# arangesh/TrackMPNN

Hardware: AMD Instinct MI355X
Metric: graph_edges_per_sec_fwd_bwd (higher is better)
Workload: dtype f32; 1 GPU; C2 KITTI Car/RRC-shaped rolling windows: 7 frames, D_t~clip(Poisson(6),1,20), F=8 (2d), H=64, K=0, diff; 1 fwd per frame + 1 bwd per window; 16384 windows/GPU batched block-diagonally (64 distinct seeds tiled); windows_per_gpu=16384, rows_final=6762496, parallelism=sequence-dp1

## Files before the change

### trackmpnn_amd/csrc/gru_fwd.hip

```cpp
#include "gru_common.h"

namespace tmpnn {

template <int CT, int XMODE>
__global__ __launch_bounds__(256, 2) void k_gru_fwd(GruFwdArgs a) {
    const int wave = threadIdx.x >> 6, lane = threadIdx.x & 63;
    const int c = lane & 31, half = lane >> 5;
    const int r0 = (blockIdx.x * 4 + wave) * 32;
    if (r0 >= a.R) return;
    const int H = a.H, H3 = 3 * a.H;
    const int col0 = blockIdx.y * (32 * CT);
    const int li = min(r0 + c, a.R - 1);
    const int row = a.rows[li];

    f32x16 acc_r[CT], acc_z[CT], acc_in[CT], acc_hn[CT];
#pragma unroll
    for (int t = 0; t < CT; ++t)
#pragma unroll
        for (int i = 0; i < 16; ++i) { acc_r[t][i] = 0.f; acc_z[t][i] = 0.f; acc_in[t][i] = 0.f; acc_hn[t][i] = 0.f; }

    for (int kt = 0; kt < a.IN / 32; ++kt) {
        const int f0 = kt * 32 + half * 16;
        float av[16];
        load_x16<XMODE>(a, li, row, f0, av);
// ... 463 lines not shown
    float* sBias = reinterpret_cast<float*>(next_item + 4);
    for (int i = threadIdx.x; i < 32; i += WPB * 64) {
        const int f = cw0 + i;
        sBias[i] = a.b_ih[f] + a.b_hh[f];
        sBias[32 + i] = a.b_ih[H + f] + a.b_hh[H + f];
        sBias[64 + i] = a.b_ih[2 * H + f];
        sBias[96 + i] = a.b_hh[2 * H + f];
        sBias[128 + i] = a.logit_part ? a.w_head[f] : 0.f;
    }
    if (threadIdx.x == 0) *next_item = 0;
    __syncthreads();
    const int wave = threadIdx.x >> 6, lane = threadIdx.x & 63;
    const int c = lane & 31, half = lane >> 5;
    if ((__builtin_amdgcn_readfirstlane(wave) >> 2) == 0) __builtin_amdgcn_s_setprio(2);
    const int tiles_total = (a.R + 31) / 32;
    const int per_group = (tiles_total + ngroups - 1) / ngroups;
    const int item_lo = group * per_group;
    const int item_hi = min(tiles_total, item_lo + per_group);

    int item = 0;
    if (lane == 0) item = atomicAdd(next_item, 1);
    item = __builtin_amdgcn_readfirstlane(item) + item_lo;
    if (item >= item_hi) return;
    int r0 = item * 32;
    int li = min(r0 + c, a.R - 1);
    int row = a.rows[li];
    float4 rawx[NQ4], rawh[NQ4];
    {
        const float4* xr = reinterpret_cast<const float4*>(a.msg + (size_t)(a.msg_compact ? li : row) * a.ld_msg + (H / 2) * half);
        const float4* hr = reinterpret_cast<const float4*>(a.h + (size_t)row * a.ld_h + (H / 2) * half);
#pragma unroll
        for (int i = 0; i < NQ4; ++i) rawx[i] = xr[i];
#pragma unroll
        for (int i = 0; i < NQ4; ++i) rawh[i] = hr[i];
    }
    float* stg = stg_base + wave * (32 * STG_LD);
    const uint16_t* wpi = sWi + c * KP + (H / 2) * half;
    const uint16_t* wph = sWh + c * KP + (H / 2) * half;

    for (;;) {
        int nitem = 0;
        if (lane == 0) nitem = atomicAdd(next_item, 1);
        nitem = __builtin_amdgcn_readfirstlane(nitem) + item_lo;
        const bool nvalid = nitem < item_hi;
        const int nr0 = nvalid ? nitem * 32 : r0;
        const int nli = min(nr0 + c, a.R - 1);
        const int nrow = a.rows[nli];
        f32x16 acc_r, acc_z, acc_hn, acc_in;
#pragma unroll
        for (int i = 0; i < 16; ++i) { acc_r[i] = 0.f; acc_z[i] = 0.f; acc_hn[i] = 0.f; acc_in[i] = 0.f; }
        Split8 b[NKB];
#pragma unroll
        for (int kb = 0; kb < NKB; ++kb) b[kb] = split8(rawx[2 * kb], rawx[2 * kb + 1]);
        if (nvalid) {
            const float4* xr = reinterpret_cast<const float4*>(a.msg + (size_t)(a.msg_compact ? nli : nrow) * a.ld_msg + (H / 2) * half);
#pragma unroll
            for (int i = 0; i < NQ4; ++i) rawx[i] = xr[i];
        }
#pragma unroll
        for (int kb = 0; kb < NKB; ++kb) {
#pragma unroll
            for (int g = 0; g < 3; ++g) {
                const uint16_t* wp = wpi + (g * 32) * KP + 8 * kb;
                const uint4 w1 = *reinterpret_cast<const uint4*>(wp);
                const uint4 w2 = *reinterpret_cast<const uint4*>(wp + NC * KP);
                const uint4 w3 = *reinterpret_cast<const uint4*>(wp + 2 * NC * KP);
                if (g == 0) acc_r = mfma_x6(w1, w2, w3, b[kb], acc_r);
                else if (g == 1) acc_z = mfma_x6(w1, w2, w3, b[kb], acc_z);
                else acc_in = mfma_x6(w1, w2, w3, b[kb], acc_in);
            }
        }
#pragma unroll
        for (int kb = 0; kb < NKB; ++kb) b[kb] = split8(rawh[2 * kb], rawh[2 * kb + 1]);
        if (nvalid) {
            const float4* hr = reinterpret_cast<const float4*>(a.h + (size_t)nrow * a.ld_h + (H / 2) * half);
#pragma unroll
            for (int i = 0; i < NQ4; ++i) rawh[i] = hr[i];
        }
#pragma unroll
        for (int kb = 0; kb < NKB; ++kb) {
#pragma unroll
            for (int g = 0; g < 3; ++g) {
                const uint16_t* wp = wph + (g * 32) * KP + 8 * kb;
                const uint4 w1 = *reinterpret_cast<const uint4*>(wp);
                const uint4 w2 = *reinterpret_cast<const uint4*>(wp + NC * KP);
                const uint4 w3 = *reinterpret_cast<const uint4*>(wp + 2 * NC * KP);
                if (g == 0) acc_r = mfma_x6(w1, w2, w3, b[kb], acc_r);
                else if (g == 1) acc_z = mfma_x6(w1, w2, w3, b[kb], acc_z);
                else acc_hn = mfma_x6(w1, w2, w3, b[kb], acc_hn);
            }
        }
        float4 hp4[4];
#pragma unroll
        for (int q = 0; q < 4; ++q)
            hp4[q] = *reinterpret_cast<const float4*>(a.h + (size_t)row * a.ld_h + cw0 + 8 * q + 4 * half);
        f32x16 outv;
#pragma unroll
        for (int q = 0; q < 4; ++q) {
            const float4 br = *reinterpret_cast<const float4*>(sBias + 8 * q + 4 * half);
            const float4 bz = *reinterpret_cast<const float4*>(sBias + 32 + 8 * q + 4 * half);
            const float4 bi = *reinterpret_cast<const float4*>(sBias + 64 + 8 * q + 4 * half);
            const float4 bh = *reinterpret_cast<const float4*>(sBias + 96 + 8 * q + 4 * half);
            const float brv[4] = {br.x, br.y, br.z, br.w}, bzv[4] = {bz.x, bz.y, bz.z, bz.w};
            const float biv[4] = {bi.x, bi.y, bi.z, bi.w}, bhv[4] = {bh.x, bh.y, bh.z, bh.w};
            const float hp[4] = {hp4[q].x, hp4[q].y, hp4[q].z, hp4[q].w};
#pragma unroll
            for (int i = 0; i < 4; ++i) {
                const int reg = 4 * q + i;
                const float ro = sigmoidf_(acc_r[reg] + brv[i]);
                const float zo = sigmoidf_(acc_z[reg] + bzv[i]);
                const float ho = acc_hn[reg] + bhv[i];
                const float no = tanhf_(acc_in[reg] + biv[i] + ro * ho);
                outv[reg] = (1.0f - zo) * no + zo * hp[i];
                acc_r[reg] = ro; acc_z[reg] = zo; acc_hn[reg] = ho; acc_in[reg] = no;
            }
        }
        if (a.logit_part) {
            float p = 0.f;
#pragma unroll
            for (int q = 0; q < 4; ++q) {
                const float4 w = *reinterpret_cast<const float4*>(sBias + 128 + 8 * q + 4 * half);
                p += outv[4 * q] * w.x + outv[4 * q + 1] * w.y + outv[4 * q + 2] * w.z + outv[4 * q + 3] * w.w;
            }
            p += __shfl_xor(p, 32);
            if (half == 0 && r0 + c < a.R) a.logit_part[(size_t)cwb * a.part_stride + row] = p;
        }
        stage_store32(stg, c, half, lane, outv, a.h_out, a.ld_out, cw0, row, r0, a.R);
        if (a.gates) {
            stage_store32<true>(stg, c, half, lane, acc_r, a.gates, H, cw0, row, r0, a.R);
            stage_store32<true>(stg, c, half, lane, acc_z, a.gates + a.gate_plane, H, cw0, row, r0, a.R);
            stage_store32<true>(stg, c, half, lane, acc_in, a.gates + 2 * a.gate_plane, H, cw0, row, r0, a.R);
            stage_store32<true>(stg, c, half, lane, acc_hn, a.gates + 3 * a.gate_plane, H, cw0, row, r0, a.R);
        }
        if (!nvalid) break;
        r0 = nr0; li = nli; row = nrow;
    }
}

#define FT_MARK(i) do { } while (0)
struct FwdTiles { const int32_t* t_row; const int32_t* t_loc; const int32_t* t_dptr; const int32_t* t_dets; int T; int zs_hn; };
static constexpr int TCAP = 24, TP_LD = 100;
static constexpr int TP_AREA = TCAP * TP_LD;

__device__ __forceinline__ uint32_t lds_addr_g(const void* p) {
    return (uint32_t)(uintptr_t)(const __attribute__((address_space(3))) char*)(const char*)p;
}
__device__ __forceinline__ void glds16_g(const void* gsrc, uint32_t lds_wave_base) {
    unsigned keep;
    lds_wave_base = __builtin_amdgcn_readfirstlane(lds_wave_base);
    asm volatile("s_mov_b32 %0, m0\n\ts_mov_b32 m0, %2\n\ts_nop 0\n\tglobal_load_lds_dwordx4 %1, off\n\ts_mov_b32 m0, %0"
                 : "=&s"(keep) : "v"(gsrc), "s"(lds_wave_base) : "memory");
}

struct TiledIdx { int row, loc, det, nd; };
__device__ __forceinline__ TiledIdx tiled_idx(const FwdTiles& tl, int R, int t, int c, int lane) {
    TiledIdx x;
    const int li = min(32 * t + c, R - 1);
    x.row = tl.t_row[li];
    x.loc = tl.t_loc[li];
    const int dp0 = tl.t_dptr[t];
    x.nd = tl.t_dptr[t + 1] - dp0;
    x.det = lane < x.nd ? tl.t_dets[dp0 + lane] : 0;
    return x;
}
template <int H>
__device__ __forceinline__ void tiled_stage_p(const GruFwdArgs& a, const TiledIdx& x, int cw0, int lane, uint32_t area) {
    const int nchunk = x.nd * 25;
#pragma unroll 1
    for (int i0 = 0; i0 < nchunk; i0 += 64) {
        const int idx = i0 + lane;
        const int j = idx / 25, rem = idx - 25 * j;
        const int j0 = i0 / 25;
        const int d0 = __builtin_amdgcn_readlane(x.det, j0), d1 = __builtin_amdgcn_readlane(x.det, j0 + 1);
        const int d2 = __builtin_amdgcn_readlane(x.det, j0 + 2), d3 = __builtin_amdgcn_readlane(x.det, min(j0 + 3, 63));
        const int dj = j - j0;
        const int det = dj == 0 ? d0 : dj == 1 ? d1 : dj == 2 ? d2 : d3;
        if (idx < nchunk && rem < 24)
            glds16_g(a.msg + (size_t)det * a.ld_msg + (rem >> 3) * H + cw0 + 4 * (rem & 7), area + 16u * i0);
    }
}

template <int H>
__device__ __forceinline__ void tiled_stage_p2(const GruFwdArgs& a, const TiledIdx& x, int cw0, int lane, uint32_t area) {
    const int sub = lane >= 25 ? 1 : 0, rem = lane - 25 * sub;
    const int goff = (rem >> 3) * H + cw0 + 4 * (rem & 7);
    const bool lane_on = rem < 24 && lane < 49;
#pragma unroll 1
    for (int k = 0; 2 * k < x.nd; ++k) {
        const int d0 = __builtin_amdgcn_readlane(x.det, 2 * k), d1 = __builtin_amdgcn_readlane(x.det, min(2 * k + 1, 63));
        const int det = sub ? d1 : d0;
        if (lane_on && 2 * k + sub < x.nd) glds16_g(a.msg + (size_t)det * a.ld_msg + goff, area + 800u * k);
    }
}

#define FT_STAGE_P tiled_stage_p2
template <int H, int WPB, bool ZS = false>
__global__ __launch_bounds__(WPB * 64, ZS ? 3 : 1) void k_gru_fwd_split_tiled(GruFwdArgs a, FwdTiles tl) {
    extern __shared__ float lds[];
    constexpr int H3 = 3 * H, KP = H + 8, NKB = H / 16, CW = H / 32, NQ4 = H / 8;
    uint16_t* sW = reinterpret_cast<uint16_t*>(lds);
    if constexpr (!ZS)
    for (int i = threadIdx.x; i < H * H3 / 4; i += WPB * 64) {
        const int k = i / (H3 / 4), j0 = (i % (H3 / 4)) * 4;
        const float4 w = *reinterpret_cast<const float4*>(a.whh_t + (size_t)k * H3 + j0);
        const float wv[4] = {w.x, w.y, w.z, w.w};
#pragma unroll
        for (int e = 0; e < 4; ++e) {
            uint16_t q1, q2, q3;
            split1(wv[e], q1, q2, q3);
            sW[(0 * H3 + j0 + e) * KP + k] = q1;
            sW[(1 * H3 + j0 + e) * KP + k] = q2;
            sW[(2 * H3 + j0 + e) * KP + k] = q3;
        }
    }
    float* area_base = reinterpret_cast<float*>(sW + (ZS ? 0 : 3 * H3 * KP));
    int* next_item = reinterpret_cast<int*>(area_base + WPB * TP_AREA);
    float* sBias = reinterpret_cast<float*>(next_item + 4);
    for (int i = threadIdx.x; i < H; i += WPB * 64) {
        sBias[i] = a.b_ih[i] + a.b_hh[i];
        sBias[H + i] = a.b_ih[H + i] + a.b_hh[H + i];
        sBias[2 * H + i] = a.b_ih[2 * H + i];
        sBias[3 * H + i] = a.b_hh[2 * H + i];
        sBias[4 * H + i] = a.logit_part ? a.w_head[i] : 0.f;
    }
    if (threadIdx.x == 0) *next_item = 0;
    __syncthreads();
    const int wave = threadIdx.x >> 6, lane = threadIdx.x & 63;
    const int c = lane & 31, half = lane >> 5;
    {
        const int grp = __builtin_amdgcn_readfirstlane(wave) >> 2;
        if (grp == 0) __builtin_amdgcn_s_setprio(3);
        else if (grp == 1) __builtin_amdgcn_s_setprio(2);
        else if (grp == 2) __builtin_amdgcn_s_setprio(1);
    }
    const int items_total = tl.T * CW;
    const int per_block = (items_total + gridDim.x - 1) / gridDim.x;
    const int item_lo = blockIdx.x * per_block;
    const int item_hi = min(items_total, item_lo + per_block);

    int item = 0;
    if (lane == 0) item = atomicAdd(next_item, 1);
    item = __builtin_amdgcn_readfirstlane(item) + item_lo;
    if (item >= item_hi) return;
    int cw0 = (item % CW) * 32;
    int t = item / CW;
    TiledIdx ix = tiled_idx(tl, a.R, t, c, lane);
    float* stg = area_base + wave * TP_AREA;
    const uint32_t area = lds_addr_g(stg);
    if (ix.nd <= TCAP) FT_STAGE_P<H>(a, ix, cw0, lane, area);
    float4 raw[NQ4];
    if constexpr (!ZS) {
        const float4* xr = reinterpret_cast<const float4*>(a.h + (size_t)ix.row * a.ld_h + (H / 2) * half);
#pragma unroll
        for (int i = 0; i < NQ4; ++i) raw[i] = xr[i];
    }

    for (;;) {
        int nitem = 0;
        if (lane == 0) nitem = atomicAdd(next_item, 1);
        nitem = __builtin_amdgcn_readfirstlane(nitem) + item_lo;
        const bool nvalid = nitem < item_hi;
        const int ncw0 = (nitem % CW) * 32;
        const int nt = nvalid ? nitem / CW : t;
        const int r0 = 32 * t;
        const int row = ix.row;
        const bool staged = ix.nd <= TCAP;
        Split8 b[NKB];
        if constexpr (!ZS) {
#pragma unroll
            for (int kb = 0; kb < NKB; ++kb) b[kb] = split8(raw[2 * kb], raw[2 * kb + 1]);
        }
        const TiledIdx nix = tiled_idx(tl, a.R, nt, c, lane);
        if constexpr (!ZS) {
            if (nvalid) {
                const float4* xr = reinterpret_cast<const float4*>(a.h + (size_t)nix.row * a.ld_h + (H / 2) * half);
#pragma unroll
                for (int i = 0; i < NQ4; ++i) raw[i] = xr[i];
            }
        }
        f32x16 acc_r, acc_z, acc_hn, acc_in;
#pragma unroll
        for (int i = 0; i < 16; ++i) { acc_r[i] = 0.f; acc_z[i] = 0.f; acc_hn[i] = 0.f; }
        if constexpr (!ZS) {
            const uint16_t* wp0 = sW + (cw0 + c) * KP + (H / 2) * half;
#pragma unroll
            for (int kb = 0; kb < NKB; ++kb) {
                const uint16_t* wp = wp0 + 8 * kb;
#pragma unroll
                for (int g = 0; g < 3; ++g) {
                    const uint4 w1 = *reinterpret_cast<const uint4*>(wp + (g * H) * KP);
                    const uint4 w2 = *reinterpret_cast<const uint4*>(wp + (H3 + g * H) * KP);
                    const uint4 w3 = *reinterpret_cast<const uint4*>(wp + (2 * H3 + g * H) * KP);
                    if (g == 0) acc_r = mfma_x6(w1, w2, w3, b[kb], acc_r);
                    else if (g == 1) acc_z = mfma_x6(w1, w2, w3, b[kb], acc_z);
                    else acc_hn = mfma_x6(w1, w2, w3, b[kb], acc_hn);
                }
            }
        }
        if (staged) {
            if (!ZS && nvalid) {
                if constexpr (NQ4 == 8) asm volatile("s_waitcnt vmcnt(8)" ::: "memory");
                else asm volatile("s_waitcnt vmcnt(4)" ::: "memory");
            } else {
                asm volatile("s_waitcnt vmcnt(0)" ::: "memory");
            }
        }
        float4 hp4[4];
        if constexpr (ZS) {
#pragma unroll
            for (int q = 0; q < 4; ++q) hp4[q] = make_float4(0.f, 0.f, 0.f, 0.f);
        } else {
#pragma unroll
            for (int q = 0; q < 4; ++q)
                hp4[q] = *reinterpret_cast<const float4*>(a.h + (size_t)row * a.ld_h + cw0 + 8 * q + 4 * half);
        }
        f32x16 outv;
        {
            float4 gs[4], gd[4], hs[4], hd[4];
            const int ls = ix.loc & 0xFFFF, ld_ = ix.loc >> 16;
            const int sdet = __shfl(ix.det, ls, 64), ddet = __shfl(ix.det, ld_, 64);
            const float* ps0 = a.msg + (size_t)sdet * a.ld_msg + cw0 + 4 * half;
            const float* pd0 = a.msg + (size_t)ddet * a.ld_msg + cw0 + 4 * half;
            if (staged) {
                const float* ls0 = stg + ls * TP_LD + 4 * half;
                const float* ld0 = stg + ld_ * TP_LD + 4 * half;
#pragma unroll
                for (int q = 0; q < 4; ++q) gs[q] = *reinterpret_cast<const float4*>(ls0 + 8 * q);
#pragma unroll
                for (int q = 0; q < 4; ++q) gd[q] = *reinterpret_cast<const float4*>(ld0 + 8 * q);
#pragma unroll
                for (int q = 0; q < 4; ++q) hs[q] = *reinterpret_cast<const float4*>(ls0 + 32 + 8 * q);
#pragma unroll
                for (int q = 0; q < 4; ++q) hd[q] = *reinterpret_cast<const float4*>(ld0 + 32 + 8 * q);
            } else {
#pragma unroll
                for (int q = 0; q < 4; ++q) gs[q] = *reinterpret_cast<const float4*>(ps0 + 8 * q);
#pragma unroll
                for (int q = 0; q < 4; ++q) gd[q] = *reinterpret_cast<const float4*>(pd0 + 8 * q);
#pragma unroll
                for (int q = 0; q < 4; ++q) hs[q] = *reinterpret_cast<const float4*>(ps0 + H + 8 * q);
#pragma unroll
                for (int q = 0; q < 4; ++q) hd[q] = *reinterpret_cast<const float4*>(pd0 + H + 8 * q);
            }
            __builtin_amdgcn_sched_barrier(0);
#pragma unroll
            for (int q = 0; q < 4; ++q) {
                const float4 b4 = *reinterpret_cast<const float4*>(sBias + cw0 + 8 * q + 4 * half);
                acc_r[4 * q + 0] = acc_r[4 * q + 0] + (gs[q].x - gd[q].x) + b4.x;
                acc_r[4 * q + 1] = acc_r[4 * q + 1] + (gs[q].y - gd[q].y) + b4.y;
                acc_r[4 * q + 2] = acc_r[4 * q + 2] + (gs[q].z - gd[q].z) + b4.z;
                acc_r[4 * q + 3] = acc_r[4 * q + 3] + (gs[q].w - gd[q].w) + b4.w;
            }
            __builtin_amdgcn_sched_barrier(0);
            if (staged) {
                const float* ls0 = stg + ls * TP_LD + 4 * half + 64;
                const float* ld0 = stg + ld_ * TP_LD + 4 * half + 64;
#pragma unroll
                for (int q = 0; q < 4; ++q) gs[q] = *reinterpret_cast<const float4*>(ls0 + 8 * q);
#pragma unroll
                for (int q = 0; q < 4; ++q) gd[q] = *reinterpret_cast<const float4*>(ld0 + 8 * q);
            } else {
#pragma unroll
                for (int q = 0; q < 4; ++q) gs[q] = *reinterpret_cast<const float4*>(ps0 + 2 * H + 8 * q);
#pragma unroll
                for (int q = 0; q < 4; ++q) gd[q] = *reinterpret_cast<const float4*>(pd0 + 2 * H + 8 * q);
            }
            __builtin_amdgcn_sched_barrier(0);
#pragma unroll
            for (int q = 0; q < 4; ++q) {
                const float4 b4 = *reinterpret_cast<const float4*>(sBias + H + cw0 + 8 * q + 4 * half);
                acc_z[4 * q + 0] = acc_z[4 * q + 0] + (hs[q].x - hd[q].x) + b4.x;
                acc_z[4 * q + 1] = acc_z[4 * q + 1] + (hs[q].y - hd[q].y) + b4.y;
                acc_z[4 * q + 2] = acc_z[4 * q + 2] + (hs[q].z - hd[q].z) + b4.z;
                acc_z[4 * q + 3] = acc_z[4 * q + 3] + (hs[q].w - hd[q].w) + b4.w;
            }
#pragma unroll
            for (int q = 0; q < 4; ++q) {
                const float4 b4 = *reinterpret_cast<const float4*>(sBias + 2 * H + cw0 + 8 * q + 4 * half);
                acc_in[4 * q + 0] = (gs[q].x - gd[q].x) + b4.x;
                acc_in[4 * q + 1] = (gs[q].y - gd[q].y) + b4.y;
                acc_in[4 * q + 2] = (gs[q].z - gd[q].z) + b4.z;
                acc_in[4 * q + 3] = (gs[q].w - gd[q].w) + b4.w;
            }
#pragma unroll
            for (int q = 0; q < 4; ++q) {
                const float4 b4h = *reinterpret_cast<const float4*>(sBias + 3 * H + cw0 + 8 * q + 4 * half);
                const float bh[4] = {b4h.x, b4h.y, b4h.z, b4h.w};
                const float hp[4] = {hp4[q].x, hp4[q].y, hp4[q].z, hp4[q].w};
#pragma unroll
                for (int i = 0; i < 4; ++i) {
                    const int reg = 4 * q + i;
                    const float ro = sigmoidf_(acc_r[reg]);
                    const float zo = sigmoidf_(acc_z[reg]);
                    const float ho = acc_hn[reg] + bh[i];
                    const float no = tanhf_(gru_n_preact(acc_in[reg], ro, ho));
                    outv[reg] = (1.0f - zo) * no + zo * hp[i];
                    acc_r[reg] = ro; acc_z[reg] = zo; acc_hn[reg] = ho; acc_in[reg] = no;
                }
            }
        }
        if (a.logit_part) {
            float p = 0.f;
#pragma unroll
            for (int q = 0; q < 4; ++q) {
                const float4 w = *reinterpret_cast<const float4*>(sBias + 4 * H + cw0 + 8 * q + 4 * half);
                p += outv[4 * q] * w.x + outv[4 * q + 1] * w.y + outv[4 * q + 2] * w.z + outv[4 * q + 3] * w.w;
            }
            p += __shfl_xor(p, 32);
            if (half == 0 && r0 + c < a.R) a.logit_part[(size_t)(cw0 / 32) * a.part_stride + row] = p;
        }
        asm volatile("s_waitcnt lgkmcnt(0)" ::: "memory");
        stage_store32(stg, c, half, lane, outv, a.h_out, a.ld_out, cw0, row, r0, a.R);
        if (a.gates) {
            stage_store32<true>(stg, c, half, lane, acc_r, a.gates, H, cw0, row, r0, a.R);
            stage_store32<true>(stg, c, half, lane, acc_z, a.gates + a.gate_plane, H, cw0, row, r0, a.R);
            stage_store32<true>(stg, c, half, lane, acc_in, a.gates + 2 * a.gate_plane, H, cw0, row, r0, a.R);
            if (!ZS || tl.zs_hn) stage_store32<true>(stg, c, half, lane, acc_hn, a.gates + 3 * a.gate_plane, H, cw0, row, r0, a.R);
        }
        if (!nvalid) break;
        cw0 = ncw0; t = nt; ix = nix;
        if (ix.nd <= TCAP) FT_STAGE_P<H>(a, ix, cw0, lane, area);
    }
}


static constexpr int T16_CAP = 12;
static constexpr int T16_AREA = T16_CAP * TP_LD;

__device__ __forceinline__ f32x4 mfma16_x6(const uint4& a1, const uint4& a2, const uint4& a3, const Split8& b, f32x4 c) {
    c = __builtin_amdgcn_mfma_f32_16x16x32_bf16(__builtin_bit_cast(bf16x8, a3), __builtin_bit_cast(bf16x8, b.p1), c, 0, 0, 0);
    c = __builtin_amdgcn_mfma_f32_16x16x32_bf16(__builtin_bit_cast(bf16x8, a1), __builtin_bit_cast(bf16x8, b.p3), c, 0, 0, 0);
    c = __builtin_amdgcn_mfma_f32_16x16x32_bf16(__builtin_bit_cast(bf16x8, a2), __builtin_bit_cast(bf16x8, b.p2), c, 0, 0, 0);
    c = __builtin_amdgcn_mfma_f32_16x16x32_bf16(__builtin_bit_cast(bf16x8, a2), __builtin_bit_cast(bf16x8, b.p1), c, 0, 0, 0);
    c = __builtin_amdgcn_mfma_f32_16x16x32_bf16(__builtin_bit_cast(bf16x8, a1), __builtin_bit_cast(bf16x8, b.p2), c, 0, 0, 0);
    c = __builtin_amdgcn_mfma_f32_16x16x32_bf16(__builtin_bit_cast(bf16x8, a1), __builtin_bit_cast(bf16x8, b.p1), c, 0, 0, 0);
    return c;
}
struct T16Idx { int row, loc, dp0, nd, det; };
__device__ __forceinline__ T16Idx t16_idx(const FwdTiles& tl, int R, int t, int n) {
    T16Idx x;
    const int li = min(16 * t + n, R - 1);
    x.row = tl.t_row[li];
    x.loc = tl.t_loc[li];
    typedef int i32x2u __attribute__((ext_vector_type(2), aligned(4)));
    const i32x2u dp = *reinterpret_cast<const i32x2u*>(tl.t_dptr + t);
    x.dp0 = dp[0];
    x.nd = dp[1] - dp[0];
    x.det = 0;
    return x;
}
__device__ __forceinline__ int t16_det(const FwdTiles& tl, const T16Idx& x, int lane) {
    return tl.t_dets[x.dp0 + min(lane, max(x.nd - 1, 0))];
}
__device__ __forceinline__ void nt_store4(float* p, const f32x4& v) {
    __builtin_nontemporal_store(v, reinterpret_cast<f32x4*>(p));
}

template <int H, int WPB>
__global__ __launch_bounds__(WPB * 64) void k_gru_fwd_split_t16(GruFwdArgs a, FwdTiles tl) {
    extern __shared__ float lds[];
    constexpr int H3 = 3 * H, NKS = H / 32, CW = H / 32;
    uint16_t* sW = reinterpret_cast<uint16_t*>(lds);
    constexpr int PLANE = H3 * 8;
    for (int i = threadIdx.x; i < H * H3 / 4; i += WPB * 64) {
        const int k = i / (H3 / 4), j0 = (i % (H3 / 4)) * 4;
        const float4 w = *reinterpret_cast<const float4*>(a.whh_t + (size_t)k * H3 + j0);
        const float wv[4] = {w.x, w.y, w.z, w.w};
        const int kgp = k / (8 * NKS), sp = (k / 8) % NKS, jp = k & 7;
#pragma unroll
        for (int e = 0; e < 4; ++e) {
            uint16_t q1, q2, q3;
            split1(wv[e], q1, q2, q3);
            const int o = ((sp * 4 + kgp) * H3 + j0 + e) * 8 + jp;
            sW[o] = q1;
            sW[NKS * 4 * PLANE + o] = q2;
            sW[2 * NKS * 4 * PLANE + o] = q3;
        }
    }
    float* area_base = reinterpret_cast<float*>(sW + 3 * NKS * 4 * PLANE);
    int* next_item = reinterpret_cast<int*>(area_base + WPB * T16_AREA);
    float* sBias = reinterpret_cast<float*>(next_item + 4);
    for (int i = threadIdx.x; i < H; i += WPB * 64) {
        sBias[i] = a.b_ih[i] + a.b_hh[i];
        sBias[H + i] = a.b_ih[H + i] + a.b_hh[H + i];
        sBias[2 * H + i] = a.b_ih[2 * H + i];
        sBias[3 * H + i] = a.b_hh[2 * H + i];
        sBias[4 * H + i] = a.logit_part ? a.w_head[i] : 0.f;
    }
    if (threadIdx.x == 0) *next_item = 0;
    __syncthreads();
    const int wave = threadIdx.x >> 6, lane = threadIdx.x & 63;
    const int n = lane & 15, kg = lane >> 4;
    const int items_total = tl.T * CW;
    const int per_block = (items_total + gridDim.x - 1) / gridDim.x;
    const int item_lo = blockIdx.x * per_block;
    const int item_hi = min(items_total, item_lo + per_block);
    auto claim = [&]() {
        int v = 0;
        if (lane == 0) v = atomicAdd(next_item, 1);
        return __builtin_amdgcn_readfirstlane(v) + item_lo;
    };
    int item = claim();
    if (item >= item_hi) return;
    int nitem = claim();
    const int last_t = (item_hi - 1) / CW;
    int t = item / CW, cw0 = (item % CW) * 32;
    int nt = nitem < item_hi ? nitem / CW : last_t;
    T16Idx ix = t16_idx(tl, a.R, t, n);
    T16Idx nix = t16_idx(tl, a.R, nt, n);
    ix.det = t16_det(tl, ix, lane);
    float* stg = area_base + wave * T16_AREA;
    const uint32_t area = lds_addr_g(stg);
    auto stage_p = [&](const T16Idx& x, int c0) {
        if (x.nd <= T16_CAP) tiled_stage_p<H>(a, TiledIdx{x.row, x.loc, x.det, x.nd}, c0, lane, area);
    };
    stage_p(ix, cw0);
    float4 raw[2 * NKS];
    {
        const float4* xr = reinterpret_cast<const float4*>(a.h + (size_t)ix.row * a.ld_h + 8 * NKS * kg);
#pragma unroll
        for (int i = 0; i < 2 * NKS; ++i) raw[i] = xr[i];
    }
    f32x4 hp4[2];
#pragma unroll
    for (int ct = 0; ct < 2; ++ct)
        hp4[ct] = *reinterpret_cast<const f32x4*>(a.h + (size_t)ix.row * a.ld_h + cw0 + 16 * ct + 4 * kg);
    const int nst = __builtin_amdgcn_readfirstlane(2 + (a.gates ? 8 : 0) + (a.logit_part ? 1 : 0));
    bool first = true;
    const bool lo = n < 8;
    const int colw = 16 * (n >> 3) + 4 * kg;
    for (;;) {
        const bool nvalid = nitem < item_hi;
        const int ncw0 = (nitem % CW) * 32;
        const int row = ix.row;
        const bool live = 16 * t + n < a.R;
        const bool staged = ix.nd <= T16_CAP;
        Split8 b[NKS];
#pragma unroll
        for (int s_ = 0; s_ < NKS; ++s_) b[s_] = split8(raw[2 * s_], raw[2 * s_ + 1]);
        {
            const float4* xr = reinterpret_cast<const float4*>(a.h + (size_t)nix.row * a.ld_h + 8 * NKS * kg);
#pragma unroll
            for (int i = 0; i < 2 * NKS; ++i) raw[i] = xr[i];
        }
        nix.det = t16_det(tl, nix, lane);
        const int n2item = claim();
        const int n2t = n2item < item_hi ? n2item / CW : last_t;
        const T16Idx n2ix = t16_idx(tl, a.R, n2t, n);
        __builtin_amdgcn_sched_barrier(0);
        f32x4 acc[3][2];
#pragma unroll
        for (int g = 0; g < 3; ++g)
#pragma unroll
            for (int ct = 0; ct < 2; ++ct)
#pragma unroll
                for (int i = 0; i < 4; ++i) acc[g][ct][i] = 0.f;
        {
            const uint16_t* wp0 = sW + (kg * H3 + cw0 + n) * 8;
#pragma unroll
            for (int s_ = 0; s_ < NKS; ++s_)
#pragma unroll
                for (int g = 0; g < 3; ++g)
#pragma unroll
                    for (int ct = 0; ct < 2; ++ct) {
                        const uint16_t* wp = wp0 + s_ * 4 * PLANE + (g * H + 16 * ct) * 8;
                        const uint4 w1 = *reinterpret_cast<const uint4*>(wp);
                        const uint4 w2 = *reinterpret_cast<const uint4*>(wp + NKS * 4 * PLANE);
                        const uint4 w3 = *reinterpret_cast<const uint4*>(wp + 2 * NKS * 4 * PLANE);
                        acc[g][ct] = mfma16_x6(w1, w2, w3, b[s_], acc[g][ct]);
                    }
        }
        if (first) {
            asm volatile("s_waitcnt vmcnt(0)" ::: "memory");
        } else if constexpr (NKS == 2) {
// ... 474 lines not shown
```

Measured before the change: 745.6 million graph-edges/s.

## Deepen software pipeline in tiled GRU forward with two-ahead index prefetch

Restructures the persistent work loop of the tiled GRU forward kernel to claim work items two ahead and prefetch the next tile's row, loc, det and dptr indices with inline-asm global loads tracked by explicit vmcnt waits. The previous-hidden slice hp4 is now taken from the already-loaded raw input registers through permlane32_swap instead of a separate global reload. The next tile's raw h loads are issued after the MFMA phase, and waits are counted against the number of outstanding stores. This aims to hide index and hidden-state load latency, at the cost of fragile hand-counted vmcnt accounting and more live registers.

```diff
diff --git a/trackmpnn_amd/csrc/gru_fwd.hip b/trackmpnn_amd/csrc/gru_fwd.hip
--- a/trackmpnn_amd/csrc/gru_fwd.hip
+++ b/trackmpnn_amd/csrc/gru_fwd.hip
@@ -639,6 +639,37 @@
                  : "=&s"(keep) : "v"(gsrc), "s"(lds_wave_base) : "memory");
 }
 
+typedef int i32x2u __attribute__((ext_vector_type(2)));
+template <int OFF>
+__device__ __forceinline__ void pl_load16(f32x4& d, const void* p) {
+    asm volatile("global_load_dwordx4 %0, %1, off offset:%2" : "=v"(d) : "v"(p), "i"(OFF) : "memory");
+}
+__device__ __forceinline__ void pl_load8(i32x2u& d, const void* p) {
+    asm volatile("global_load_dwordx2 %0, %1, off" : "=v"(d) : "v"(p) : "memory");
+}
+__device__ __forceinline__ void pl_load4(int& d, const void* p) {
+    asm volatile("global_load_dword %0, %1, off" : "=v"(d) : "v"(p) : "memory");
+}
+template <int N>
+__device__ __forceinline__ void pl_wait() {
+    static_assert(N >= 0 && N <= 63, "vmcnt is a 6-bit field");
+    asm volatile("s_waitcnt vmcnt(%0)" ::"i"(N) : "memory");
+}
+template <int ADD>
+__device__ __forceinline__ void wait_stores(int nst) {
+    switch (nst) {
+        case 4: pl_wait<ADD + 4>(); break;
+        case 5: pl_wait<ADD + 5>(); break;
+        case 16: pl_wait<ADD + 16>(); break;
+        case 17: pl_wait<ADD + 17>(); break;
+        case 20: pl_wait<ADD + 20>(); break;
+        case 21: pl_wait<ADD + 21>(); break;
+        default: pl_wait<0>(); break;
+    }
+}
+
+__device__ __forceinline__ void gather_wait(float4& v) { asm volatile("" : "+v"(v.x), "+v"(v.y), "+v"(v.z), "+v"(v.w)); }
+
 struct TiledIdx { int row, loc, det, nd; };
 __device__ __forceinline__ TiledIdx tiled_idx(const FwdTiles& tl, int R, int t, int c, int lane) {
     TiledIdx x;
@@ -725,45 +756,68 @@
     const int item_lo = blockIdx.x * per_block;
     const int item_hi = min(items_total, item_lo + per_block);
 
-    int item = 0;
-    if (lane == 0) item = atomicAdd(next_item, 1);
-    item = __builtin_amdgcn_readfirstlane(item) + item_lo;
+    auto claim = [&]() {
+        int v = 0;
+        if (lane == 0) v = atomicAdd(next_item, 1);
+        return __builtin_amdgcn_readfirstlane(v) + item_lo;
+    };
+    const int item = claim();
     if (item >= item_hi) return;
+    int nitem = claim(), n2item = claim();
     int cw0 = (item % CW) * 32;
     int t = item / CW;
+    bool nvalid = nitem < item_hi;
+    int ncw0 = (nitem % CW) * 32, nt = nvalid ? nitem / CW : t;
+    int n2t = n2item < item_hi ? n2item / CW : nt;
     TiledIdx ix = tiled_idx(tl, a.R, t, c, lane);
+    ix.nd = __builtin_amdgcn_readfirstlane(ix.nd);
+    int na_row, na_loc, na_dp0, na_nd;
+    {
+        const int li = min(32 * nt + c, a.R - 1);
+        na_row = tl.t_row[li];
+        na_loc = tl.t_loc[li];
+        na_dp0 = __builtin_amdgcn_readfirstlane(tl.t_dptr[nt]);
+        na_nd = __builtin_amdgcn_readfirstlane(tl.t_dptr[nt + 1]) - na_dp0;
+    }
     float* stg = area_base + wave * TP_AREA;
     const uint32_t area = lds_addr_g(stg);
     if (ix.nd <= TCAP) FT_STAGE_P<H>(a, ix, cw0, lane, area);
-    float4 raw[NQ4];
+    f32x4 raw[NQ4];
     if constexpr (!ZS) {
-        const float4* xr = reinterpret_cast<const float4*>(a.h + (size_t)ix.row * a.ld_h + (H / 2) * half);
+        const f32x4* xr = reinterpret_cast<const f32x4*>(a.h + (size_t)ix.row * a.ld_h + (H / 2) * half);
 #pragma unroll
         for (int i = 0; i < NQ4; ++i) raw[i] = xr[i];
     }
+    const int nst = __builtin_amdgcn_readfirstlane((a.logit_part ? 1 : 0) +
+                                                   4 * (1 + (a.gates ? (ZS ? 3 + (tl.zs_hn ? 1 : 0) : 4) : 0)));
+    bool drain_in = true;
+    asm volatile("" : "+v"(ix.row), "+v"(ix.loc), "+v"(ix.det), "+v"(na_row), "+v"(na_loc));
+    if constexpr (!ZS) {
+#pragma unroll
+        for (int i = 0; i < NQ4; ++i) asm volatile("" : "+v"(raw[i]));
+    }
 
     for (;;) {
-        int nitem = 0;
-        if (lane == 0) nitem = atomicAdd(next_item, 1);
-        nitem = __builtin_amdgcn_readfirstlane(nitem) + item_lo;
-        const bool nvalid = nitem < item_hi;
-        const int ncw0 = (nitem % CW) * 32;
-        const int nt = nvalid ? nitem / CW : t;
         const int r0 = 32 * t;
         const int row = ix.row;
         const bool staged = ix.nd <= TCAP;
+        const bool drain_out = !staged || r0 + 32 > a.R;
         Split8 b[NKB];
+        f32x4 hp4[4];
         if constexpr (!ZS) {
 #pragma unroll
-            for (int kb = 0; kb < NKB; ++kb) b[kb] = split8(raw[2 * kb], raw[2 * kb + 1]);
-        }
-        const TiledIdx nix = tiled_idx(tl, a.R, nt, c, lane);
-        if constexpr (!ZS) {
-            if (nvalid) {
-                const float4* xr = reinterpret_cast<const float4*>(a.h + (size_t)nix.row * a.ld_h + (H / 2) * half);
-#pragma unroll
-                for (int i = 0; i < NQ4; ++i) raw[i] = xr[i];
-            }
+            for (int kb = 0; kb < NKB; ++kb)
+                b[kb] = split8(make_float4(raw[2 * kb].x, raw[2 * kb].y, raw[2 * kb].z, raw[2 * kb].w),
+                               make_float4(raw[2 * kb + 1].x, raw[2 * kb + 1].y, raw[2 * kb + 1].z, raw[2 * kb + 1].w));
+        }
+        i32x2u n2_dp;
+        int n2_row, n2_loc, n_det;
+        {
+            const int li = min(32 * n2t + c, a.R - 1);
+            pl_load8(n2_dp, tl.t_dptr + n2t);
+            pl_load4(n2_row, tl.t_row + li);
+            pl_load4(n2_loc, tl.t_loc + li);
+            pl_load4(n_det, tl.t_dets + na_dp0 + min(lane, max(na_nd - 1, 0)));
         }
         f32x16 acc_r, acc_z, acc_hn, acc_in;
 #pragma unroll
@@ -785,21 +839,36 @@
             }
         }
         if (staged) {
-            if (!ZS && nvalid) {
-                if constexpr (NQ4 == 8) asm volatile("s_waitcnt vmcnt(8)" ::: "memory");
-                else asm volatile("s_waitcnt vmcnt(4)" ::: "memory");
-            } else {
-                asm volatile("s_waitcnt vmcnt(0)" ::: "memory");
-            }
-        }
-        float4 hp4[4];
-        if constexpr (ZS) {
-#pragma unroll
-            for (int q = 0; q < 4; ++q) hp4[q] = make_float4(0.f, 0.f, 0.f, 0.f);
+            if (drain_in) pl_wait<0>();
+            else pl_wait<4>();
+        }
+        __builtin_amdgcn_sched_barrier(0);
+        if constexpr (!ZS) {
+#pragma unroll
+            for (int p = 0; p < NQ4 / 2; ++p)
+#pragma unroll
+                for (int i = 0; i < 4; ++i) {
+                    const auto sw = __builtin_amdgcn_permlane32_swap(__float_as_uint(raw[2 * p][i]), __float_as_uint(raw[2 * p + 1][i]),
+                                                                     false, false);
+                    if constexpr (H == 64) {
+                        hp4[p][i] = __uint_as_float(cw0 ? sw[1] : sw[0]);
+                    } else {
+                        hp4[p][i] = __uint_as_float(sw[0]);
+                        hp4[2 + p][i] = __uint_as_float(sw[1]);
+                    }
+                }
+#pragma unroll
+            for (int q = 0; q < 4; ++q) asm volatile("" : "+v"(hp4[q]));
         } else {
 #pragma unroll
-            for (int q = 0; q < 4; ++q)
-                hp4[q] = *reinterpret_cast<const float4*>(a.h + (size_t)row * a.ld_h + cw0 + 8 * q + 4 * half);
+            for (int q = 0; q < 4; ++q) hp4[q] = f32x4{0.f, 0.f, 0.f, 0.f};
+        }
+        if constexpr (!ZS) {
+            const float* xr = a.h + (size_t)na_row * a.ld_h + (H / 2) * half;
+            pl_load16<0>(raw[0], xr); pl_load16<16>(raw[1], xr); pl_load16<32>(raw[2], xr); pl_load16<48>(raw[3], xr);
+            if constexpr (NQ4 == 8) {
+                pl_load16<64>(raw[4], xr); pl_load16<80>(raw[5], xr); pl_load16<96>(raw[6], xr); pl_load16<112>(raw[7], xr);
+            }
         }
         f32x16 outv;
         {
@@ -828,6 +897,8 @@
                 for (int q = 0; q < 4; ++q) hs[q] = *reinterpret_cast<const float4*>(ps0 + H + 8 * q);
 #pragma unroll
                 for (int q = 0; q < 4; ++q) hd[q] = *reinterpret_cast<const float4*>(pd0 + H + 8 * q);
+#pragma unroll
+                for (int q = 0; q < 4; ++q) { gather_wait(gs[q]); gather_wait(gd[q]); gather_wait(hs[q]); gather_wait(hd[q]); }
             }
             __builtin_amdgcn_sched_barrier(0);
 #pragma unroll
@@ -851,6 +922,8 @@
                 for (int q = 0; q < 4; ++q) gs[q] = *reinterpret_cast<const float4*>(ps0 + 2 * H + 8 * q);
 #pragma unroll
                 for (int q = 0; q < 4; ++q) gd[q] = *reinterpret_cast<const float4*>(pd0 + 2 * H + 8 * q);
+#pragma unroll
+                for (int q = 0; q < 4; ++q) { gather_wait(gs[q]); gather_wait(gd[q]); }
             }
             __builtin_amdgcn_sched_barrier(0);
 #pragma unroll
@@ -905,8 +978,31 @@
             if (!ZS || tl.zs_hn) stage_store32<true>(stg, c, half, lane, acc_hn, a.gates + 3 * a.gate_plane, H, cw0, row, r0, a.R);
         }
         if (!nvalid) break;
-        cw0 = ncw0; t = nt; ix = nix;
-        if (ix.nd <= TCAP) FT_STAGE_P<H>(a, ix, cw0, lane, area);
+        if (drain_out) pl_wait<0>();
+        else wait_stores<ZS ? 0 : NQ4>(nst);
+        asm volatile("" : "+v"(n_det), "+v"(n2_dp), "+v"(n2_row), "+v"(n2_loc));
+        cw0 = ncw0; t = nt;
+        ix.row = na_row; ix.loc = na_loc; ix.det = n_det; ix.nd = na_nd;
+        na_row = n2_row; na_loc = n2_loc;
+        na_dp0 = __builtin_amdgcn_readfirstlane(n2_dp[0]);
+        na_nd = __builtin_amdgcn_readfirstlane(n2_dp[1]) - na_dp0;
+        nitem = n2item; nvalid = nitem < item_hi; ncw0 = (nitem % CW) * 32; nt = n2t;
+        {
+            int lane_d = lane;
+            asm volatile("" : "+v"(lane_d));
+            if (ix.nd <= TCAP) FT_STAGE_P<H>(a, ix, cw0, lane_d, area);
+        }
+        n2item = claim();
+        n2t = n2item < item_hi ? n2item / CW : nt;
+        if constexpr (!ZS) {
+            if (drain_out) pl_wait<0>();
+            else wait_stores<0>(nst);
+            if constexpr (NQ4 == 8)
+                asm volatile("" : "+v"(raw[0]), "+v"(raw[1]), "+v"(raw[2]), "+v"(raw[3]), "+v"(raw[4]), "+v"(raw[5]), "+v"(raw[6]), "+v"(raw[7]));
+            else
+                asm volatile("" : "+v"(raw[0]), "+v"(raw[1]), "+v"(raw[2]), "+v"(raw[3]));
+        }
+        drain_in = drain_out;
     }
 }
 
```

New measurement: 748.9 million graph-edges/s, median of 6. No clear change (+0.4%).

## Process all column tiles per row tile in one work item, reusing loaded hidden state

Applied to the files above, without the earlier changes.

In the non-zero-state tiled GRU forward kernel, a work item now covers a whole 32-row tile across all column halves, not one (row tile, column half) pair. The hidden-state row is loaded once and reused for every column half. The previous-h values for the blend are taken from those registers through permlane32 swaps instead of a second global load. This cuts repeated h reads and atomic work fetches, at the cost of fewer, coarser work items, a serial loop over column halves, and re-staging messages between halves.

```diff
diff --git a/trackmpnn_amd/csrc/gru_fwd.hip b/trackmpnn_amd/csrc/gru_fwd.hip
--- a/trackmpnn_amd/csrc/gru_fwd.hip
+++ b/trackmpnn_amd/csrc/gru_fwd.hip
@@ -681,6 +681,34 @@
 }
 
 #define FT_STAGE_P tiled_stage_p2
+
+__device__ __forceinline__ void ld4x4(float4* g, const float* p) {
+#pragma unroll
+    for (int q = 0; q < 4; ++q) g[q] = *reinterpret_cast<const float4*>(p + 8 * q);
+}
+
+template <int H>
+__device__ __forceinline__ void hp_from_raw(const float4* raw, int m, float4* hp4) {
+#pragma unroll
+    for (int j = 0; j < H / 16; ++j) {
+        const float av[4] = {raw[2 * j].x, raw[2 * j].y, raw[2 * j].z, raw[2 * j].w};
+        const float bv[4] = {raw[2 * j + 1].x, raw[2 * j + 1].y, raw[2 * j + 1].z, raw[2 * j + 1].w};
+        float lo[4], hi[4];
+#pragma unroll
+        for (int i = 0; i < 4; ++i) {
+            const auto r = __builtin_amdgcn_permlane32_swap(__float_as_uint(av[i]), __float_as_uint(bv[i]), false, false);
+            lo[i] = __uint_as_float(r[0]);
+            hi[i] = __uint_as_float(r[1]);
+        }
+        if constexpr (H == 64) {
+            hp4[j] = m == 0 ? make_float4(lo[0], lo[1], lo[2], lo[3]) : make_float4(hi[0], hi[1], hi[2], hi[3]);
+        } else {
+            hp4[j] = make_float4(lo[0], lo[1], lo[2], lo[3]);
+            hp4[2 + j] = make_float4(hi[0], hi[1], hi[2], hi[3]);
+        }
+    }
+}
+
 template <int H, int WPB, bool ZS = false>
 __global__ __launch_bounds__(WPB * 64, ZS ? 3 : 1) void k_gru_fwd_split_tiled(GruFwdArgs a, FwdTiles tl) {
     extern __shared__ float lds[];
@@ -720,7 +748,8 @@
         else if (grp == 1) __builtin_amdgcn_s_setprio(2);
         else if (grp == 2) __builtin_amdgcn_s_setprio(1);
     }
-    const int items_total = tl.T * CW;
+    constexpr int IPT = ZS ? CW : 1, NHALF = ZS ? 1 : CW;
+    const int items_total = tl.T * IPT;
     const int per_block = (items_total + gridDim.x - 1) / gridDim.x;
     const int item_lo = blockIdx.x * per_block;
     const int item_hi = min(items_total, item_lo + per_block);
@@ -729,8 +758,8 @@
     if (lane == 0) item = atomicAdd(next_item, 1);
     item = __builtin_amdgcn_readfirstlane(item) + item_lo;
     if (item >= item_hi) return;
-    int cw0 = (item % CW) * 32;
-    int t = item / CW;
+    int cw0 = (item % IPT) * 32;
+    int t = item / IPT;
     TiledIdx ix = tiled_idx(tl, a.R, t, c, lane);
     float* stg = area_base + wave * TP_AREA;
     const uint32_t area = lds_addr_g(stg);
@@ -747,162 +776,149 @@
         if (lane == 0) nitem = atomicAdd(next_item, 1);
         nitem = __builtin_amdgcn_readfirstlane(nitem) + item_lo;
         const bool nvalid = nitem < item_hi;
-        const int ncw0 = (nitem % CW) * 32;
-        const int nt = nvalid ? nitem / CW : t;
+        const int ncw0 = (nitem % IPT) * 32;
+        const int nt = nvalid ? nitem / IPT : t;
         const int r0 = 32 * t;
         const int row = ix.row;
         const bool staged = ix.nd <= TCAP;
-        Split8 b[NKB];
-        if constexpr (!ZS) {
-#pragma unroll
-            for (int kb = 0; kb < NKB; ++kb) b[kb] = split8(raw[2 * kb], raw[2 * kb + 1]);
-        }
-        const TiledIdx nix = tiled_idx(tl, a.R, nt, c, lane);
-        if constexpr (!ZS) {
-            if (nvalid) {
-                const float4* xr = reinterpret_cast<const float4*>(a.h + (size_t)nix.row * a.ld_h + (H / 2) * half);
-#pragma unroll
-                for (int i = 0; i < NQ4; ++i) raw[i] = xr[i];
-            }
-        }
-        f32x16 acc_r, acc_z, acc_hn, acc_in;
-#pragma unroll
-        for (int i = 0; i < 16; ++i) { acc_r[i] = 0.f; acc_z[i] = 0.f; acc_hn[i] = 0.f; }
-        if constexpr (!ZS) {
-            const uint16_t* wp0 = sW + (cw0 + c) * KP + (H / 2) * half;
-#pragma unroll
-            for (int kb = 0; kb < NKB; ++kb) {
-                const uint16_t* wp = wp0 + 8 * kb;
-#pragma unroll
-                for (int g = 0; g < 3; ++g) {
-                    const uint4 w1 = *reinterpret_cast<const uint4*>(wp + (g * H) * KP);
-                    const uint4 w2 = *reinterpret_cast<const uint4*>(wp + (H3 + g * H) * KP);
-                    const uint4 w3 = *reinterpret_cast<const uint4*>(wp + (2 * H3 + g * H) * KP);
-                    if (g == 0) acc_r = mfma_x6(w1, w2, w3, b[kb], acc_r);
-                    else if (g == 1) acc_z = mfma_x6(w1, w2, w3, b[kb], acc_z);
-                    else acc_hn = mfma_x6(w1, w2, w3, b[kb], acc_hn);
-                }
-            }
-        }
-        if (staged) {
-            if (!ZS && nvalid) {
-                if constexpr (NQ4 == 8) asm volatile("s_waitcnt vmcnt(8)" ::: "memory");
-                else asm volatile("s_waitcnt vmcnt(4)" ::: "memory");
-            } else {
-                asm volatile("s_waitcnt vmcnt(0)" ::: "memory");
-            }
-        }
-        float4 hp4[4];
-        if constexpr (ZS) {
-#pragma unroll
-            for (int q = 0; q < 4; ++q) hp4[q] = make_float4(0.f, 0.f, 0.f, 0.f);
-        } else {
-#pragma unroll
-            for (int q = 0; q < 4; ++q)
-                hp4[q] = *reinterpret_cast<const float4*>(a.h + (size_t)row * a.ld_h + cw0 + 8 * q + 4 * half);
-        }
-        f32x16 outv;
-        {
-            float4 gs[4], gd[4], hs[4], hd[4];
-            const int ls = ix.loc & 0xFFFF, ld_ = ix.loc >> 16;
-            const int sdet = __shfl(ix.det, ls, 64), ddet = __shfl(ix.det, ld_, 64);
-            const float* ps0 = a.msg + (size_t)sdet * a.ld_msg + cw0 + 4 * half;
-            const float* pd0 = a.msg + (size_t)ddet * a.ld_msg + cw0 + 4 * half;
+        TiledIdx nix;
+#pragma unroll
+        for (int m = 0; m < NHALF; ++m) {
+            int lane_t = lane;
+            if constexpr (!ZS) asm volatile("" : "+v"(lane_t));
+            const int lane = lane_t, c = lane & 31, half = lane >> 5;
+            if constexpr (!ZS) {
+                cw0 = 32 * m;
+                asm volatile("" : "+s"(cw0));
+                if (m > 0) {
+#pragma unroll
+                    for (int i = 0; i < NQ4; ++i)
+                        asm volatile("" : "+v"(raw[i].x), "+v"(raw[i].y), "+v"(raw[i].z), "+v"(raw[i].w));
+                }
+            }
+            const bool last = m == NHALF - 1;
+            Split8 b[NKB];
+            float4 hp4[4];
+            if constexpr (!ZS) {
+#pragma unroll
+                for (int kb = 0; kb < NKB; ++kb) b[kb] = split8(raw[2 * kb], raw[2 * kb + 1]);
+            }
+            if (m == 0) nix = tiled_idx(tl, a.R, nt, c, lane);
+            if constexpr (!ZS) {
+                hp_from_raw<H>(raw, m, hp4);
+                if (last && nvalid) {
+                    const float4* xr = reinterpret_cast<const float4*>(a.h + (size_t)nix.row * a.ld_h + (H / 2) * half);
+#pragma unroll
+                    for (int i = 0; i < NQ4; ++i) raw[i] = xr[i];
+                }
+            }
+            f32x16 acc_r, acc_z, acc_hn, acc_in;
+#pragma unroll
+            for (int i = 0; i < 16; ++i) { acc_r[i] = 0.f; acc_z[i] = 0.f; acc_hn[i] = 0.f; }
+            if constexpr (!ZS) {
+                const uint16_t* wp0 = sW + (cw0 + c) * KP + (H / 2) * half;
+#pragma unroll
+                for (int kb = 0; kb < NKB; ++kb) {
+                    const uint16_t* wp = wp0 + 8 * kb;
+#pragma unroll
+                    for (int g = 0; g < 3; ++g) {
+                        const uint4 w1 = *reinterpret_cast<const uint4*>(wp + (g * H) * KP);
+                        const uint4 w2 = *reinterpret_cast<const uint4*>(wp + (H3 + g * H) * KP);
+                        const uint4 w3 = *reinterpret_cast<const uint4*>(wp + (2 * H3 + g * H) * KP);
+                        if (g == 0) acc_r = mfma_x6(w1, w2, w3, b[kb], acc_r);
+                        else if (g == 1) acc_z = mfma_x6(w1, w2, w3, b[kb], acc_z);
+                        else acc_hn = mfma_x6(w1, w2, w3, b[kb], acc_hn);
+                    }
+                }
+            }
             if (staged) {
-                const float* ls0 = stg + ls * TP_LD + 4 * half;
-                const float* ld0 = stg + ld_ * TP_LD + 4 * half;
-#pragma unroll
-                for (int q = 0; q < 4; ++q) gs[q] = *reinterpret_cast<const float4*>(ls0 + 8 * q);
-#pragma unroll
-                for (int q = 0; q < 4; ++q) gd[q] = *reinterpret_cast<const float4*>(ld0 + 8 * q);
-#pragma unroll
-                for (int q = 0; q < 4; ++q) hs[q] = *reinterpret_cast<const float4*>(ls0 + 32 + 8 * q);
-#pragma unroll
-                for (int q = 0; q < 4; ++q) hd[q] = *reinterpret_cast<const float4*>(ld0 + 32 + 8 * q);
-            } else {
-#pragma unroll
-                for (int q = 0; q < 4; ++q) gs[q] = *reinterpret_cast<const float4*>(ps0 + 8 * q);
-#pragma unroll
-                for (int q = 0; q < 4; ++q) gd[q] = *reinterpret_cast<const float4*>(pd0 + 8 * q);
-#pragma unroll
-                for (int q = 0; q < 4; ++q) hs[q] = *reinterpret_cast<const float4*>(ps0 + H + 8 * q);
-#pragma unroll
-                for (int q = 0; q < 4; ++q) hd[q] = *reinterpret_cast<const float4*>(pd0 + H + 8 * q);
-            }
-            __builtin_amdgcn_sched_barrier(0);
-#pragma unroll
-            for (int q = 0; q < 4; ++q) {
-                const float4 b4 = *reinterpret_cast<const float4*>(sBias + cw0 + 8 * q + 4 * half);
-                acc_r[4 * q + 0] = acc_r[4 * q + 0] + (gs[q].x - gd[q].x) + b4.x;
-                acc_r[4 * q + 1] = acc_r[4 * q + 1] + (gs[q].y - gd[q].y) + b4.y;
-                acc_r[4 * q + 2] = acc_r[4 * q + 2] + (gs[q].z - gd[q].z) + b4.z;
-                acc_r[4 * q + 3] = acc_r[4 * q + 3] + (gs[q].w - gd[q].w) + b4.w;
-            }
-            __builtin_amdgcn_sched_barrier(0);
-            if (staged) {
-                const float* ls0 = stg + ls * TP_LD + 4 * half + 64;
-                const float* ld0 = stg + ld_ * TP_LD + 4 * half + 64;
-#pragma unroll
-                for (int q = 0; q < 4; ++q) gs[q] = *reinterpret_cast<const float4*>(ls0 + 8 * q);
-#pragma unroll
-                for (int q = 0; q < 4; ++q) gd[q] = *reinterpret_cast<const float4*>(ld0 + 8 * q);
-            } else {
-#pragma unroll
-                for (int q = 0; q < 4; ++q) gs[q] = *reinterpret_cast<const float4*>(ps0 + 2 * H + 8 * q);
-#pragma unroll
-                for (int q = 0; q < 4; ++q) gd[q] = *reinterpret_cast<const float4*>(pd0 + 2 * H + 8 * q);
-            }
-            __builtin_amdgcn_sched_barrier(0);
-#pragma unroll
-            for (int q = 0; q < 4; ++q) {
-                const float4 b4 = *reinterpret_cast<const float4*>(sBias + H + cw0 + 8 * q + 4 * half);
-                acc_z[4 * q + 0] = acc_z[4 * q + 0] + (hs[q].x - hd[q].x) + b4.x;
-                acc_z[4 * q + 1] = acc_z[4 * q + 1] + (hs[q].y - hd[q].y) + b4.y;
-                acc_z[4 * q + 2] = acc_z[4 * q + 2] + (hs[q].z - hd[q].z) + b4.z;
-                acc_z[4 * q + 3] = acc_z[4 * q + 3] + (hs[q].w - hd[q].w) + b4.w;
-            }
-#pragma unroll
-            for (int q = 0; q < 4; ++q) {
-                const float4 b4 = *reinterpret_cast<const float4*>(sBias + 2 * H + cw0 + 8 * q + 4 * half);
-                acc_in[4 * q + 0] = (gs[q].x - gd[q].x) + b4.x;
-                acc_in[4 * q + 1] = (gs[q].y - gd[q].y) + b4.y;
-                acc_in[4 * q + 2] = (gs[q].z - gd[q].z) + b4.z;
-                acc_in[4 * q + 3] = (gs[q].w - gd[q].w) + b4.w;
-            }
-#pragma unroll
-            for (int q = 0; q < 4; ++q) {
-                const float4 b4h = *reinterpret_cast<const float4*>(sBias + 3 * H + cw0 + 8 * q + 4 * half);
-                const float bh[4] = {b4h.x, b4h.y, b4h.z, b4h.w};
-                const float hp[4] = {hp4[q].x, hp4[q].y, hp4[q].z, hp4[q].w};
-#pragma unroll
-                for (int i = 0; i < 4; ++i) {
-                    const int reg = 4 * q + i;
-                    const float ro = sigmoidf_(acc_r[reg]);
-                    const float zo = sigmoidf_(acc_z[reg]);
-                    const float ho = acc_hn[reg] + bh[i];
-                    const float no = tanhf_(gru_n_preact(acc_in[reg], ro, ho));
-                    outv[reg] = (1.0f - zo) * no + zo * hp[i];
-                    acc_r[reg] = ro; acc_z[reg] = zo; acc_hn[reg] = ho; acc_in[reg] = no;
-                }
-            }
-        }
-        if (a.logit_part) {
-            float p = 0.f;
-#pragma unroll
-            for (int q = 0; q < 4; ++q) {
-                const float4 w = *reinterpret_cast<const float4*>(sBias + 4 * H + cw0 + 8 * q + 4 * half);
-                p += outv[4 * q] * w.x + outv[4 * q + 1] * w.y + outv[4 * q + 2] * w.z + outv[4 * q + 3] * w.w;
-            }
-            p += __shfl_xor(p, 32);
-            if (half == 0 && r0 + c < a.R) a.logit_part[(size_t)(cw0 / 32) * a.part_stride + row] = p;
-        }
-        asm volatile("s_waitcnt lgkmcnt(0)" ::: "memory");
-        stage_store32(stg, c, half, lane, outv, a.h_out, a.ld_out, cw0, row, r0, a.R);
-        if (a.gates) {
-            stage_store32<true>(stg, c, half, lane, acc_r, a.gates, H, cw0, row, r0, a.R);
-            stage_store32<true>(stg, c, half, lane, acc_z, a.gates + a.gate_plane, H, cw0, row, r0, a.R);
-            stage_store32<true>(stg, c, half, lane, acc_in, a.gates + 2 * a.gate_plane, H, cw0, row, r0, a.R);
-            if (!ZS || tl.zs_hn) stage_store32<true>(stg, c, half, lane, acc_hn, a.gates + 3 * a.gate_plane, H, cw0, row, r0, a.R);
+                if (!ZS && last && nvalid) {
+                    if constexpr (NQ4 == 8) asm volatile("s_waitcnt vmcnt(8)" ::: "memory");
+                    else asm volatile("s_waitcnt vmcnt(4)" ::: "memory");
+                } else {
+                    asm volatile("s_waitcnt vmcnt(0)" ::: "memory");
+                }
+            }
+            if constexpr (ZS) {
+#pragma unroll
+                for (int q = 0; q < 4; ++q) hp4[q] = make_float4(0.f, 0.f, 0.f, 0.f);
+            }
+            f32x16 outv;
+            {
+                float4 gs[4], gd[4], hs[4], hd[4];
+                const int ls = ix.loc & 0xFFFF, ld_ = ix.loc >> 16;
+                const int sdet = __shfl(ix.det, ls, 64), ddet = __shfl(ix.det, ld_, 64);
+                const float* ps0 = a.msg + (size_t)sdet * a.ld_msg + cw0 + 4 * half;
+                const float* pd0 = a.msg + (size_t)ddet * a.ld_msg + cw0 + 4 * half;
+                if (staged) { ld4x4(gs, stg + ls * TP_LD + 4 * half); ld4x4(gd, stg + ld_ * TP_LD + 4 * half); }
+                else { ld4x4(gs, ps0); ld4x4(gd, pd0); }
+                if (staged) { ld4x4(hs, stg + ls * TP_LD + 4 * half + 32); ld4x4(hd, stg + ld_ * TP_LD + 4 * half + 32); }
+                else { ld4x4(hs, ps0 + H); ld4x4(hd, pd0 + H); }
+                __builtin_amdgcn_sched_barrier(0);
+#pragma unroll
+                for (int q = 0; q < 4; ++q) {
+                    const float4 b4 = *reinterpret_cast<const float4*>(sBias + cw0 + 8 * q + 4 * half);
+                    acc_r[4 * q + 0] = acc_r[4 * q + 0] + (gs[q].x - gd[q].x) + b4.x;
+                    acc_r[4 * q + 1] = acc_r[4 * q + 1] + (gs[q].y - gd[q].y) + b4.y;
+                    acc_r[4 * q + 2] = acc_r[4 * q + 2] + (gs[q].z - gd[q].z) + b4.z;
+                    acc_r[4 * q + 3] = acc_r[4 * q + 3] + (gs[q].w - gd[q].w) + b4.w;
+                }
+                __builtin_amdgcn_sched_barrier(0);
+                if (staged) { ld4x4(gs, stg + ls * TP_LD + 4 * half + 64); ld4x4(gd, stg + ld_ * TP_LD + 4 * half + 64); }
+                else { ld4x4(gs, ps0 + 2 * H); ld4x4(gd, pd0 + 2 * H); }
+                __builtin_amdgcn_sched_barrier(0);
+#pragma unroll
+                for (int q = 0; q < 4; ++q) {
+                    const float4 b4 = *reinterpret_cast<const float4*>(sBias + H + cw0 + 8 * q + 4 * half);
+                    acc_z[4 * q + 0] = acc_z[4 * q + 0] + (hs[q].x - hd[q].x) + b4.x;
+                    acc_z[4 * q + 1] = acc_z[4 * q + 1] + (hs[q].y - hd[q].y) + b4.y;
+                    acc_z[4 * q + 2] = acc_z[4 * q + 2] + (hs[q].z - hd[q].z) + b4.z;
+                    acc_z[4 * q + 3] = acc_z[4 * q + 3] + (hs[q].w - hd[q].w) + b4.w;
+                }
+#pragma unroll
+                for (int q = 0; q < 4; ++q) {
+                    const float4 b4 = *reinterpret_cast<const float4*>(sBias + 2 * H + cw0 + 8 * q + 4 * half);
+                    acc_in[4 * q + 0] = (gs[q].x - gd[q].x) + b4.x;
+                    acc_in[4 * q + 1] = (gs[q].y - gd[q].y) + b4.y;
+                    acc_in[4 * q + 2] = (gs[q].z - gd[q].z) + b4.z;
+                    acc_in[4 * q + 3] = (gs[q].w - gd[q].w) + b4.w;
+                }
+#pragma unroll
+                for (int q = 0; q < 4; ++q) {
+                    const float4 b4h = *reinterpret_cast<const float4*>(sBias + 3 * H + cw0 + 8 * q + 4 * half);
+                    const float bh[4] = {b4h.x, b4h.y, b4h.z, b4h.w};
+                    const float hp[4] = {hp4[q].x, hp4[q].y, hp4[q].z, hp4[q].w};
+#pragma unroll
+                    for (int i = 0; i < 4; ++i) {
+                        const int reg = 4 * q + i;
+                        const float ro = sigmoidf_(acc_r[reg]);
+                        const float zo = sigmoidf_(acc_z[reg]);
+                        const float ho = acc_hn[reg] + bh[i];
+                        const float no = tanhf_(gru_n_preact(acc_in[reg], ro, ho));
+                        outv[reg] = (1.0f - zo) * no + zo * hp[i];
+                        acc_r[reg] = ro; acc_z[reg] = zo; acc_hn[reg] = ho; acc_in[reg] = no;
+                    }
+                }
+            }
+            if (a.logit_part) {
+                float p = 0.f;
+#pragma unroll
+                for (int q = 0; q < 4; ++q) {
+                    const float4 w = *reinterpret_cast<const float4*>(sBias + 4 * H + cw0 + 8 * q + 4 * half);
+                    p += outv[4 * q] * w.x + outv[4 * q + 1] * w.y + outv[4 * q + 2] * w.z + outv[4 * q + 3] * w.w;
+                }
+                p += __shfl_xor(p, 32);
+                if (half == 0 && r0 + c < a.R) a.logit_part[(size_t)(cw0 / 32) * a.part_stride + row] = p;
+            }
+            asm volatile("s_waitcnt lgkmcnt(0)" ::: "memory");
+            stage_store32(stg, c, half, lane, outv, a.h_out, a.ld_out, cw0, row, r0, a.R);
+            if (a.gates) {
+                stage_store32<true>(stg, c, half, lane, acc_r, a.gates, H, cw0, row, r0, a.R);
+                stage_store32<true>(stg, c, half, lane, acc_z, a.gates + a.gate_plane, H, cw0, row, r0, a.R);
+                stage_store32<true>(stg, c, half, lane, acc_in, a.gates + 2 * a.gate_plane, H, cw0, row, r0, a.R);
+                if (!ZS || tl.zs_hn) stage_store32<true>(stg, c, half, lane, acc_hn, a.gates + 3 * a.gate_plane, H, cw0, row, r0, a.R);
+            }
+            if (!last && staged) FT_STAGE_P<H>(a, ix, cw0 + 32, lane, area);
         }
         if (!nvalid) break;
         cw0 = ncw0; t = nt; ix = nix;
```

Result: no change. 744.5 million graph-edges/s before, 747.9 million graph-edges/s after, median of 6 (+0.5%).
